# NVlabs/ODISE

Hardware: AMD Instinct MI355X
Metric: panoptic-inference images/sec @1024x1024 (higher is better)
Workload: dtype f16

## Files before the change

odise_amd/csrc/gemm.hip:

```cpp
#include "common.h"
#include <stdlib.h>
#include <type_traits>

#ifdef ODISE_TOOLS
#define ODISE_ABLATE(g, bit) ((g).dbg & (bit))
#else
#define ODISE_ABLATE(g, bit) false
#endif

namespace odise {

struct GemmEpi {
    void* C;
    int64_t ldc;
    int c_dtype;
    const float* bias_n;
    const float* bias_m;
    const float* scale_m;
    const f16* residual;
    int64_t ldr;
    const float* rowgroup_add;
    int rows_per_group;
    int64_t ldg;
    int act;
// ... 1949 lines not shown
    };
    auto finish = [&](TileK& t) { t.kw = (t.ky * 3 + t.kx) * g.cg.Cin + t.chunk * BK; };
    auto advance = [&](TileK& t) {
        if (++t.kx == 3) {
            t.kx = 0;
            if (++t.ky == 3) { t.ky = 0; ++t.chunk; }
        }
        finish(t);
    };

    AccBlock acc[TM][TN];
#pragma unroll
    for (int i = 0; i < TM; ++i)
#pragma unroll
        for (int j = 0; j < TN; ++j) acc_zero(acc[i][j]);

    const int lrow = Frag::lrow(lane), lkq = Frag::lk(lane);
    int koff[Frag::NSTEP];
#pragma unroll
    for (int s = 0; s < Frag::NSTEP; ++s) koff[s] = (Frag::kslot(s, lkq) ^ ((lrow >> 1) & 7)) << 4;
    const int b_lane_off = (wn * WTN + lrow) * 128;
    const int a_pix0 = (wm * 4 + (lrow >> 4)) * HW_ + (lrow & 15);

    auto read_a = [&](const TileK& t, int s, f16x8 (&dst)[TM][Frag::NSTEP][Frag::PER]) {
        const char* ha = smem + HALO0 + (t.chunk & 1) * HALO_BYTES;
        const int pix = a_pix0 + t.ky * HW_ + t.kx;
        const int key = (((lrow & 15) + t.kx) >> 1) & 7;
#pragma unroll
        for (int i = 0; i < TM; ++i)
#pragma unroll
            for (int u = 0; u < Frag::PER; ++u)
                dst[i][s][u] = *reinterpret_cast<const f16x8*>(ha + (pix + (i * 2 + u) * HW_) * 128 + ((Frag::kslot(s, lkq) ^ key) << 4));
    };
    TileK t0;
    t0.ky = t0.kx = 0;
    t0.chunk = kt_begin / 9;
    finish(t0);
    TileK t1 = t0, t2;
    if (kt_begin < kt_end) {
        advance(t1);
        issue_halo(t0.chunk);
#pragma unroll
        for (int j = 0; j < JB; ++j) issue_B(j, 0, t0.kw);
        if (kt_begin + 1 < kt_end) {
#pragma unroll
            for (int j = 0; j < LB; ++j) issue_B(j, 1, t1.kw);
            wait_vmcnt<LB>();
        } else {
            wait_vmcnt<0>();
        }
    }
    t2 = t1;
    advance(t2);
    __builtin_amdgcn_s_barrier();
    TileK tc = t0;
    f16x8 af[TM][Frag::NSTEP][Frag::PER], bf[PT][Frag::NSTEP][Frag::PER];
    {
        const char* fb = smem + b_lane_off;
#pragma unroll
        for (int s = 0; s < Frag::NSTEP; ++s) {
            read_a(tc, s, af);
#pragma unroll
            for (int jj = 0; jj < PT; ++jj)
#pragma unroll
                for (int u = 0; u < Frag::PER; ++u) bf[jj][s][u] = *reinterpret_cast<const f16x8*>(fb + koff[s] + jj * 4096 + u * 2048);
        }
    }
    if (grp == 1) __builtin_amdgcn_s_barrier();

    for (int kt = kt_begin; kt < kt_end; ++kt) {
        const int cur = (kt - kt_begin) & 1;
        const bool has1 = (kt + 1) < kt_end, has2 = (kt + 2) < kt_end;
        const bool opens = tc.ky == 0 && tc.kx == 0;
        const bool halo_next = opens && (kt + 9) < kt_end;
#pragma unroll
        for (int p = 0; p < NP; ++p) {
            const int j0 = PT * p;
            if (p == 0) {
                if (has1) {
#pragma unroll
                    for (int j = LB; j < JB; ++j) issue_B(j, cur ^ 1, t1.kw);
                }
                if (halo_next) issue_halo(tc.chunk + 1);
                if (halo_next) { if (has1) wait_vmcnt<LB + H>(); else wait_vmcnt<H>(); }
                else { if (has1) wait_vmcnt<LB>(); else wait_vmcnt<0>(); }
            } else {
                if (has2) {
#pragma unroll
                    for (int j = 0; j < LB; ++j) issue_B(j, cur, t2.kw);
                }
                if (halo_next) { if (has2) wait_vmcnt<LB + H>(); else wait_vmcnt<H>(); }
                else { if (has2) wait_vmcnt<LB>(); else wait_vmcnt<0>(); }
            }
            asm volatile("s_waitcnt lgkmcnt(0)" ::: "memory");
            __builtin_amdgcn_sched_barrier(0);
            __builtin_amdgcn_s_barrier();
            __builtin_amdgcn_sched_barrier(0);
            const bool next_in_tile = (p + 1 < NP);
            const bool have_next = next_in_tile || has1;
            const char* nfb = smem + (next_in_tile ? cur : (cur ^ 1)) * B_BYTES + b_lane_off + (next_in_tile ? (j0 + PT) * 4096 : 0);
            __builtin_amdgcn_s_setprio(1);
#pragma unroll
            for (int s = 0; s < Frag::NSTEP; ++s) {
#pragma unroll
                for (int jj = 0; jj < PT; ++jj)
#pragma unroll
                    for (int i = 0; i < TM; ++i) mma_step(acc[i][j0 + jj], bf[jj][s], af[i][s]);
                if (have_next) {
                    if (!next_in_tile) read_a(t1, s, af);
#pragma unroll
                    for (int jj = 0; jj < PT; ++jj)
#pragma unroll
                        for (int u = 0; u < Frag::PER; ++u) bf[jj][s][u] = *reinterpret_cast<const f16x8*>(nfb + koff[s] + jj * 4096 + u * 2048);
                }
            }
            __builtin_amdgcn_s_setprio(0);
            __builtin_amdgcn_sched_barrier(0);
            __builtin_amdgcn_s_barrier();
            __builtin_amdgcn_sched_barrier(0);
        }
        tc = t1;
        t1 = t2;
        advance(t2);
    }
    if (grp == 0) __builtin_amdgcn_s_barrier();
    asm volatile("s_waitcnt vmcnt(0) lgkmcnt(0)" ::: "memory");
    __syncthreads();
    gemm_epilogue<BM, BN, WAVES_M, WAVES_N, epi_wave_rows(BM, BN, WAVES_M, halo_lds_bytes(BN)), true, true, true,
                  epi16_rows_if_enabled(BM, BN, WAVES_M, halo_lds_bytes(BN)), false, halo_lds_bytes(BN)>(g, acc, smem, m0, n0, z, zb, split);
}

template <int BN>
__global__ void __launch_bounds__(256, 2) conv3_halo4_kernel(GemmArgs g) {
    constexpr int BM = 256, BK = 64, WAVES_M = 4, WAVES_N = 1;
    constexpr int TM = 2, TN = BN / 32;
    constexpr int JB = BN / 32;
    constexpr int HW_ = 18, HPIX = HW_ * HW_;
    constexpr int HGROUPS = (HPIX + 7) / 8;
    constexpr int H = 11;
    constexpr int B_BYTES = BN * BK * 2;
    constexpr int HALO0 = 2 * B_BYTES;
    extern __shared__ __attribute__((aligned(16))) char smem[];

    const int tid = threadIdx.x;
    const int lane = tid & 63;
    const int wave = __builtin_amdgcn_readfirstlane(tid >> 6);
    const int wm = wave;
    const int hi = lane >> 5, l31 = lane & 31;
    int bx, by;
    {
        const int nbx = gridDim.x, nb = gridDim.x * gridDim.y;
        const int bid = blockIdx.y * nbx + blockIdx.x;
        const int q = nb >> 3, r = nb & 7;
        const int xcd = bid & 7, idx = bid >> 3;
        const int logical = (xcd < r ? xcd * (q + 1) : r * (q + 1) + (xcd - r) * q) + idx;
        by = logical / nbx;
        bx = logical - by * nbx;
    }
    const int m0 = by * BM;
    const int n0 = bx * BN;
    const int z = blockIdx.z;
    const bool split = g.splitk > 1;
    const int zb = 0;
    const int nk_total = g.K / BK;
    int kt_begin = 0, kt_end = nk_total;
    if (split) {
        kt_begin = z * g.ktiles_per_split;
        kt_end = kt_begin + g.ktiles_per_split;
        if (kt_end > nk_total) kt_end = nk_total;
    }
    const f16* Wb = g.W;
    const int per_img = g.cg.halo_tx * g.cg.halo_ty;
    const int img = by / per_img, pr = by - img * per_img;
    const int py0 = (pr / g.cg.halo_tx) * 16 - 1, px0 = (pr % g.cg.halo_tx) * 16 - 1;
    const f16* Ab = g.A + (int64_t)img * g.cg.H * g.cg.W * g.cg.Cin;

    int h_off[H];
#pragma unroll
    for (int h = 0; h < H; ++h) {
        const int group = h * 4 + wave;
        const int hp = group * 8 + (lane >> 3);
        h_off[h] = -1;
        if (group < HGROUPS && hp < HPIX) {
            const int hy = hp / HW_, hx = hp - hy * HW_;
            const int iy = py0 + hy, ix = px0 + hx;
            const int up = g.cg.ups ? 1 : 0;
            if ((unsigned)iy < (unsigned)(g.cg.H << up) && (unsigned)ix < (unsigned)(g.cg.W << up))
                h_off[h] = ((iy >> up) * g.cg.W + (ix >> up)) * g.cg.Cin + (((lane & 7) ^ ((hx >> 1) & 7)) << 3);
        }
    }
    auto issue_halo = [&](int chunk) {
#pragma unroll
        for (int h = 0; h < H; ++h) {
            const int group = h * 4 + wave;
            const f16* src = h_off[h] >= 0 ? Ab + h_off[h] + chunk * BK : g.zeros;
            glds16(src, smem + HALO0 + (group < HGROUPS ? group : HGROUPS) * 1024);
        }
    };
    const int rb = wave * 8 + (lane >> 3);
    const int ls = (lane & 7) ^ ((rb >> 1) & 7);
    const int64_t b_off0 = (int64_t)(n0 + rb) * g.ldw + ls * 8;
    auto issue_B = [&](int stage, int kw) {
#pragma unroll
        for (int j = 0; j < JB; ++j) {
            const bool ok = (n0 + rb + 32 * j) < g.N;
            const f16* src = ok ? Wb + b_off0 + (int64_t)(32 * j) * g.ldw + kw : g.zeros;
            glds16(src, smem + stage * B_BYTES + (32 * j + wave * 8) * 128);
        }
    };

    AccBlock acc[TM][TN];
#pragma unroll
    for (int i = 0; i < TM; ++i)
#pragma unroll
        for (int j = 0; j < TN; ++j) acc_zero(acc[i][j]);

    const int lrow = Frag::lrow(lane), lkq = Frag::lk(lane);
    int koff[Frag::NSTEP];
#pragma unroll
    for (int s = 0; s < Frag::NSTEP; ++s) koff[s] = (Frag::kslot(s, lkq) ^ ((lrow >> 1) & 7)) << 4;
    const int b_lane_off = lrow * 128;
    const int a_pix0 = (wm * 4 + (lrow >> 4)) * HW_ + (lrow & 15);

    int ky = 0, kx = 0, chunk = kt_begin / 9;
    if (kt_begin < kt_end) {
        issue_halo(chunk);
        issue_B(0, chunk * BK);
    }
    for (int kt = kt_begin; kt < kt_end; ++kt) {
        const int cur = (kt - kt_begin) & 1;
        asm volatile("s_waitcnt vmcnt(0)" ::: "memory");
        __builtin_amdgcn_s_barrier();
        int nky = ky, nkx = kx + 1, nchunk = chunk;
        if (nkx == 3) { nkx = 0; if (++nky == 3) { nky = 0; ++nchunk; } }
        const bool more = kt + 1 < kt_end;
        if (more) issue_B(cur ^ 1, (nky * 3 + nkx) * g.cg.Cin + nchunk * BK);
        const char* ha = smem + HALO0;
        const char* fb = smem + cur * B_BYTES + b_lane_off;
        const int pix = a_pix0 + ky * HW_ + kx;
        const int key = (((lrow & 15) + kx) >> 1) & 7;
        f16x8 af[2][TM][Frag::PER], bf[2][TN][Frag::PER];
        auto read_frags = [&](int s, int b) {
#pragma unroll
            for (int u = 0; u < Frag::PER; ++u) {
#pragma unroll
                for (int i = 0; i < TM; ++i) af[b][i][u] = *reinterpret_cast<const f16x8*>(ha + (pix + (i * 2 + u) * HW_) * 128 + ((Frag::kslot(s, lkq) ^ key) << 4));
#pragma unroll
                for (int j = 0; j < TN; ++j) bf[b][j][u] = *reinterpret_cast<const f16x8*>(fb + koff[s] + j * 4096 + u * 2048);
            }
        };
        read_frags(0, 0);
#pragma unroll
        for (int s = 0; s < Frag::NSTEP; ++s) {
            if (s + 1 < Frag::NSTEP) read_frags(s + 1, (s + 1) & 1);
            __builtin_amdgcn_sched_barrier(0);
#pragma unroll
            for (int j = 0; j < TN; ++j)
#pragma unroll
                for (int i = 0; i < TM; ++i) mma_step(acc[i][j], bf[s & 1][j], af[s & 1][i]);
            __builtin_amdgcn_sched_barrier(0);
        }
        if (more && nchunk != chunk) {
            asm volatile("s_waitcnt lgkmcnt(0)" ::: "memory");
            __builtin_amdgcn_s_barrier();
            issue_halo(nchunk);
        }
        ky = nky; kx = nkx; chunk = nchunk;
    }
    asm volatile("s_waitcnt vmcnt(0) lgkmcnt(0)" ::: "memory");
    __syncthreads();
    gemm_epilogue<BM, BN, WAVES_M, WAVES_N, epi_wave_rows(BM, BN, WAVES_M, halo4_lds_bytes(BN)), true, true, true,
                  epi16_rows_if_enabled(BM, BN, WAVES_M, halo4_lds_bytes(BN)), false, halo4_lds_bytes(BN)>(g, acc, smem, m0, n0, z, zb, split);
}

__global__ void __launch_bounds__(256) splitk_reduce_kernel(const float* __restrict__ ws, int splitk, int M, int N, GemmEpi e) {
    const int CH = (N + 7) / 8;
    const int64_t total = (int64_t)M * CH;
    const bool vec = (N & 3) == 0;
    for (int64_t idx = (int64_t)blockIdx.x * blockDim.x + threadIdx.x; idx < total; idx += (int64_t)gridDim.x * blockDim.x) {
        const int m = (int)(idx / CH);
        const int n = (int)(idx - (int64_t)m * CH) * 8;
        const int nv = (N - n) < 8 ? (N - n) : 8;
        float v[8];
#pragma unroll
        for (int i = 0; i < 8; ++i) v[i] = 0.f;
        if (vec && nv == 8) {
            for (int s = 0; s < splitk; ++s) {
                const float4* w = reinterpret_cast<const float4*>(ws + ((int64_t)s * M + m) * N + n);
                const float4 a = w[0], b = w[1];
                v[0] += a.x; v[1] += a.y; v[2] += a.z; v[3] += a.w;
                v[4] += b.x; v[5] += b.y; v[6] += b.z; v[7] += b.w;
            }
        } else {
            for (int s = 0; s < splitk; ++s) {
                const float* w = ws + ((int64_t)s * M + m) * N + n;
                for (int i = 0; i < nv; ++i) v[i] += w[i];
            }
        }
        if (e.fast && n + 8 <= N) epi_fast8(e, v, m, n, 0);
        else epi_store8(e, v, m, n, N, 0);
    }
}

static int launch_tile_kernel(odise_hip_ctx* ctx, void (*kern)(GemmArgs), LdsAttrOnce& once, dim3 grid, int threads, int lds, const GemmArgs& g) {
    if (lds > 65536) ODISE_TRY(ensure_dyn_lds(ctx, once, (const void*)kern, lds));
    hipLaunchKernelGGL(kern, grid, dim3(threads), lds, ctx->stream, g);
    ODISE_CHECK_HIP(hipGetLastError());
    if (g.splitk > 1) {
        const int64_t total = (int64_t)g.M * ceil_div(g.N, 8);
        const int blocks = (int)std::min<int64_t>(ceil_div(total, 256), 2048);
        hipLaunchKernelGGL(splitk_reduce_kernel, dim3(blocks), dim3(256), 0, ctx->stream, g.ws, g.splitk, g.M, g.N, g.epi);
        ODISE_CHECK_HIP(hipGetLastError());
    }
    return ODISE_OK;
}
static dim3 gemm_grid(const GemmArgs& g, int BM, int BN, int batch) {
    return dim3((unsigned)ceil_div(g.N, BN), (unsigned)ceil_div(g.M, BM), (unsigned)(g.splitk > 1 ? g.splitk : batch));
}
static dim3 halo_grid(const GemmArgs& g, int BN) {
    const int n_img = g.M / (g.cg.OH * g.cg.OW);
    return dim3((unsigned)ceil_div(g.N, BN), (unsigned)(n_img * g.cg.halo_tx * g.cg.halo_ty), (unsigned)(g.splitk > 1 ? g.splitk : 1));
}

template <int BM, int BN, int WAVES_M, int WAVES_N, bool CONV>
static int launch_gemm_t(odise_hip_ctx* ctx, GemmArgs& g, int batch) {
    constexpr int lds = plain_lds_bytes(BM, BN, WAVES_M);
    static_assert(epi_lds_bytes(BM, BN, WAVES_M, epi_wave_rows(BM, BN, WAVES_M, lds)) <= lds, "epilogue staging exceeds the LDS request");
    static LdsAttrOnce once;
    return launch_tile_kernel(ctx, gemm_kernel<BM, BN, WAVES_M, WAVES_N, CONV>, once, gemm_grid(g, BM, BN, batch), 64 * WAVES_M * WAVES_N, lds, g);
}

template <int BM, int BN, int WAVES_N, int PT, bool CONV>
static int launch_gemm_pp(odise_hip_ctx* ctx, GemmArgs& g, int batch) {
    constexpr int lds = pp_lds_bytes(BM, BN, 8 / WAVES_N);
    static_assert(epi_lds_bytes(BM, BN, 8 / WAVES_N, epi_wave_rows(BM, BN, 8 / WAVES_N, lds)) <= lds, "epilogue staging exceeds the LDS request");
    static_assert(lds > 65536, "the ping-pong tiles always opt in to dynamic LDS");
    static LdsAttrOnce once;
    return launch_tile_kernel(ctx, gemm_pp_kernel<BM, BN, WAVES_N, PT, CONV>, once, gemm_grid(g, BM, BN, batch), 512, lds, g);
}

template <int BM, int BN, int WAVES_N, int PT, bool CONV>
static int launch_gemm_pp2(odise_hip_ctx* ctx, GemmArgs& g, int batch) {
    static_assert((BN / WAVES_N / 32) % PT == 0, "whole phases");
    constexpr int lds = pp_lds_bytes(BM, BN, 8 / WAVES_N);
    static_assert(lds > 65536, "the ping-pong tiles always opt in to dynamic LDS");
    static LdsAttrOnce once;
    return launch_tile_kernel(ctx, gemm_pp2_kernel<BM, BN, WAVES_N, PT, CONV>, once, gemm_grid(g, BM, BN, batch), 512, lds, g);
}

template <int BN, int PT>
static int launch_conv3_halo(odise_hip_ctx* ctx, GemmArgs& g) {
    constexpr int lds = halo_lds_bytes(BN);
    static_assert(epi_lds_bytes(256, BN, 4, epi_wave_rows(256, BN, 4, lds)) <= lds, "epilogue staging exceeds the LDS request");
    static_assert(lds > 65536, "the halo tiles always opt in to dynamic LDS");
    static LdsAttrOnce once;
    return launch_tile_kernel(ctx, conv3_halo_kernel<BN, PT>, once, halo_grid(g, BN), 512, lds, g);
}

template <int BN>
static int launch_conv3_halo4(odise_hip_ctx* ctx, GemmArgs& g) {
    constexpr int lds = halo4_lds_bytes(BN);
    static_assert(2 * lds <= 160 * 1024, "two blocks must fit a CU's LDS");
    static_assert(epi_lds_bytes(256, BN, 4, epi_wave_rows(256, BN, 4, lds)) <= lds, "epilogue staging exceeds the LDS request");
    static_assert(lds > 65536, "the halo tiles always opt in to dynamic LDS");
    static LdsAttrOnce once;
    return launch_tile_kernel(ctx, conv3_halo4_kernel<BN>, once, halo_grid(g, BN), 256, lds, g);
}

static int g_gemm_debug = 0;
enum SelectFlag : int {
    kFlagNoPingPong = 2,
    kFlagNo512x128 = 16,
    kFlagLaunchLog = 32,
    kFlagNoHalo = 64,
    kFlagForcePP2 = 512,
    kFlagNoPP2 = 1024,
    kFlagNoHalo4 = 2048,
    kFlagBlockEpilogue = 32768,
    kFlagNoHaloUpsample = 131072,
};
static int g_conv_flags = 0;

enum Tile : int {
    kTile128x128 = 0, kTile64x128 = 1, kTile64x64 = 2, kTile256x320 = 3, kTile256x256 = 4, kTile256x128 = 5, kTile512x128 = 6,
    kTileHalo256 = 7, kTileHalo128 = 8, kTileHalo128x4 = 9, kNumTiles = 10
};
static bool is_halo_tile(int t) { return t >= kTileHalo256 && t <= kTileHalo128x4; }
static bool has_pingpong_form(int t) { return t == kTile256x320 || t == kTile256x256 || t == kTile512x128; }
static const int kTileBM[kNumTiles] = {128, 64, 64, 256, 256, 256, 512, 256, 256, 256};
static const int kTileBN[kNumTiles] = {128, 128, 64, 320, 256, 128, 128, 256, 128, 128};

struct TileCost {
    double t_ktile, t_fixed;
    int slots_per_cu;
};
static const TileCost kTileCost[kNumTiles] = {
    {1.45, 6.0, 2},
    {1.25, 3.5, 3},
    {1.06, 2.6, 4},
    {2.65, 15.0, 1},
    {2.10, 15.0, 1},
    {1.42, 6.0, 1},
    {2.25, 12.0, 1},
    {1.47, 22.5, 1},
    {1.12, 9.0, 1},
    {1.70, 12.0, 2},
};
static const TileCost kTileCostPP[2] = {
    {2.00, 16.0, 1},
    {1.56, 10.0, 1},
};
static const TileCost kTileCostConv512 = {2.5, 16.0, 1};
static const TileCost kTileCostPPConv256 = {1.49, 25.5, 1};
static thread_local int g_last_tile = -1;
static int env_gemm_flags() {
#ifdef ODISE_TOOLS
    static int v = -1;
    if (v < 0) {
        const char* e = getenv("ODISE_GEMM_FLAGS");
        v = e ? atoi(e) : 0;
    }
    return v;
#else
    return 0;
#endif
}

template <bool CONV>
static int launch_gemm_select(odise_hip_ctx* ctx, GemmArgs& g, int batch, int force_tile, int force_split, unsigned tile_mask);

template <bool CONV>
static int launch_gemm(odise_hip_ctx* ctx, GemmArgs& g, int batch, int force_tile, int force_split, unsigned tile_mask = ~0u) {
    LaunchProbe* pr = probe_match(ctx, CONV, g.M, g.N, g.K);
    if (pr && CONV && g.cg.ups) pr = nullptr;
    if (pr) {
        hipStreamCaptureStatus st = hipStreamCaptureStatusNone;
        if (hipStreamIsCapturing(ctx->stream, &st) != hipSuccess || st != hipStreamCaptureStatusNone) pr = nullptr;
    }
    if (!pr) return launch_gemm_select<CONV>(ctx, g, batch, force_tile, force_split, tile_mask);
    const int i = pr->n;
    const bool started = hipEventRecord(pr->ev[2 * i], ctx->stream) == hipSuccess;
    const int rc = launch_gemm_select<CONV>(ctx, g, batch, force_tile, force_split, tile_mask);
    if (started && hipEventRecord(pr->ev[2 * i + 1], ctx->stream) == hipSuccess) pr->n = i + 1;
    else { (void)hipGetLastError(); pr->armed = false; }
    return rc;
}

static int select_flags() { return g_conv_flags | env_gemm_flags(); }
template <bool CONV>
static int launch_gemm_select(odise_hip_ctx* ctx, GemmArgs& g, int batch, int force_tile, int force_split, unsigned tile_mask) {
    const int64_t cus = ctx->cu_count;
    const int nk = (int)ceil_div(g.K, 64);
    bool halo_ok = false;
    int64_t halo_patches = 0;
    if (CONV) {
        const int up = g.cg.ups ? 1 : 0;
        halo_ok = g.cg.KH == 3 && g.cg.KW == 3 && g.cg.stride == 1 && g.cg.pad_t == 1 && g.cg.pad_l == 1 && g.cg.Cin % 64 == 0 &&
                  g.cg.OH == (g.cg.H << up) && g.cg.OW == (g.cg.W << up) && batch == 1 && !(up && (select_flags() & kFlagNoHaloUpsample));
        g.cg.halo_tx = (int)ceil_div(g.cg.OW, 16);
        g.cg.halo_ty = (int)ceil_div(g.cg.OH, 16);
        halo_patches = (int64_t)(g.M / (g.cg.OH * g.cg.OW)) * g.cg.halo_tx * g.cg.halo_ty;
    }
    auto blocks = [&](int t) {
        return (is_halo_tile(t) ? halo_patches : ceil_div(g.M, kTileBM[t])) * ceil_div(g.N, kTileBN[t]) * (int64_t)batch;
    };
    int tile = kTile64x64, best_split = 1;
    double best = 1e30;
    const int flags = select_flags();
    const bool pp_base = !(flags & kFlagNoPingPong) && g.K % 64 == 0 && (!CONV || g.cg.Cin % 64 == 0);
    const bool pp_ok = pp_base && !(CONV && g.cg.ups);
    for (int t = 0; t < kNumTiles; ++t) {
        if (force_tile >= 0 && force_tile < kNumTiles && t != force_tile) continue;
        if (!((tile_mask >> t) & 1)) continue;
        if (t == kTile512x128 && (!pp_ok || (flags & kFlagNo512x128))) continue;
        if (is_halo_tile(t) && (!halo_ok || !pp_base || (flags & kFlagNoHalo))) continue;
        if (t == kTileHalo128x4 && (flags & kFlagNoHalo4)) continue;
        if (t == kTileHalo128x4 && force_tile < 0 && g.N > 128) continue;
        const TileCost& tc = (CONV && pp_ok && t == kTile256x256) ? kTileCostPPConv256 :
                             (pp_ok && (t == kTile256x320 || t == kTile256x256)) ? kTileCostPP[t - kTile256x320] :
                             (CONV && t == kTile512x128) ? kTileCostConv512 : kTileCost[t];
        if (force_tile < 0) {
            if (kTileBM[t] > 64 && g.M <= kTileBM[t] / 2) continue;
            if (kTileBN[t] > 64 && g.N <= kTileBN[t] / 2 && t != kTile64x64) continue;
        }
        const int64_t nb = blocks(t);
        const int64_t slots = cus * tc.slots_per_cu;
        const int max_split = (batch == 1) ? std::max(1, std::min(nk / 2, 32)) : 1;
        for (int sp = 1; sp <= max_split; ++sp) {
            if (force_split > 0 && sp != std::min(force_split, std::max(1, nk))) continue;
            if (sp > 1 && (size_t)sp * g.M * g.N * sizeof(float) > ctx->ws_bytes) break;
            const int per = is_halo_tile(t) ? (int)ceil_div(nk / 9, sp) * 9 : (int)ceil_div(nk, sp);
            const int eff_sp = (int)ceil_div(nk, per);
            const int64_t nblk = nb * eff_sp;
            const int64_t rounds = ceil_div(nblk, slots);
            const double fill_last = (double)(nblk - (rounds - 1) * slots) / (double)slots;
            double t_us = per * tc.t_ktile * ((double)(rounds - 1) + 0.55 + 0.45 * fill_last) + (double)rounds * tc.t_fixed;
            if (eff_sp > 1) t_us += 4.0 + ((2.0 * eff_sp * 4.0 + 2.0) * (double)g.M * g.N) / 6.0e6;
            if (t_us < best) { best = t_us; tile = t; best_split = eff_sp; }
        }
    }
    if (force_tile >= 0 && force_tile < kNumTiles && !(force_tile == kTile512x128 && !pp_ok) && !(is_halo_tile(force_tile) && !(halo_ok && pp_base)))
        tile = force_tile;
    g.splitk = 1;
    g.ktiles_per_split = nk;
    if (force_split > 0 && batch == 1) best_split = std::min(force_split, nk);
    if (best_split > 1 && batch == 1) {
        g.ktiles_per_split = is_halo_tile(tile) ? (int)ceil_div(nk / 9, best_split) * 9 : (int)ceil_div(nk, best_split);
        g.splitk = (int)ceil_div(nk, g.ktiles_per_split);
        ODISE_REQUIRE((size_t)g.splitk * g.M * g.N * sizeof(float) <= ctx->ws_bytes, "gemm: split-K workspace too small");
    }
    g_last_tile = tile | (best_split << 8);
    if (ctx->launch_log) launch_log_push(ctx, LaunchRec{(int)CONV, g.M, g.N, g.K, tile, g.splitk});
    if (flags & kFlagLaunchLog) {
        fprintf(stderr, "GEMMLOG conv=%d M=%d N=%d K=%d batch=%d cin=%d kh=%d h=%d w=%d stride=%d ups=%d tile=%d split=%d pp=%d\n", (int)CONV, g.M, g.N,
                g.K, batch, g.cg.Cin, g.cg.KH, g.cg.H, g.cg.W, g.cg.stride, g.cg.ups, tile, best_split, (int)pp_ok);
    }
    g.ws = (float*)ctx->ws;
    {
        const GemmEpi& e = g.epi;
        const int esz = e.c_dtype == ODISE_F16 ? 2 : 4;
        const int out_vec = (e.geglu ? 4 : 8) * esz;
        auto aligned = [](const void* p, int64_t ld_elems, int64_t stride_elems, int elem, int bytes) {
            return ((uintptr_t)p % bytes) == 0 && (ld_elems * elem) % bytes == 0 && (stride_elems * elem) % bytes == 0;
        };
        bool ok = aligned(e.C, e.ldc, e.strideC, esz, out_vec);
        ok = ok && (!e.residual || (!e.geglu && aligned(e.residual, e.ldr, e.strideR, 2, 16)));
        ok = ok && (!e.bias_n || ((uintptr_t)e.bias_n & 15) == 0);
        ok = ok && (!e.rowgroup_add || (((uintptr_t)e.rowgroup_add & 15) == 0 && e.ldg % 4 == 0));
        ok = ok && (!e.geglu || e.act == ODISE_ACT_NONE);
        g.epi.fast = ok ? 1 : 0;
        const int n_out = e.geglu ? g.N / 2 : g.N;
        g.epi.f16path = (ok && e.c_dtype == ODISE_F16 && g.N % 8 == 0 && n_out % 8 == 0 && aligned(e.C, e.ldc, e.strideC, 2, 16) &&
                         (!e.residual || aligned(e.residual, e.ldr, e.strideR, 2, 8))) ? 1 : 0;
    }
    if (g.epi.ln_part || g.epi.ln_final || g.epi.ln_stats_out) {
        ODISE_REQUIRE(!CONV && (tile == kTile256x256 || tile == kTile256x128) && g.splitk == 1 && g.epi.f16path && !g.epi.geglu && batch == 1 &&
                          (!g.epi.ln_stats_out || (tile == kTile256x256 && g.N % kLnPartCols == 0)),
                      "gemm_ln: M=%d N=%d K=%d cannot take the folded-LayerNorm path", g.M, g.N, g.K);
    }
    g.stats_blocks = 0;
    if (g.epi.gn_stats) {
        const int ohw = CONV ? g.cg.OH * g.cg.OW : 0;
        const bool pp2_used = (tile == kTile256x256) && pp_ok && ((flags & kFlagForcePP2) || (!(flags & kFlagNoPP2) && CONV));
        bool ok = CONV && g.splitk == 1 && g.epi.fast && g.N % 8 == 0 &&
                  (is_halo_tile(tile) || (tile == kTile512x128 && pp_ok && !(flags & kFlagForcePP2)) || pp2_used);
        if (ok && is_halo_tile(tile)) g.stats_blocks = g.cg.halo_tx * g.cg.halo_ty;
        else if (ok && ohw % kTileBM[tile] == 0) g.stats_blocks = ohw / kTileBM[tile];
        else ok = false;
        if (!ok) { g.epi.gn_stats = nullptr; g.stats_blocks = 0; }
    }
    g.zeros = (const f16*)ctx->zeros;
    g.epi_block = (flags & kFlagBlockEpilogue) ? 1 : 0;
#ifdef ODISE_TOOLS
    static const int freeze_k = (getenv("ODISE_GEMM_FREEZE_K") ? 16 : 0) | (getenv("ODISE_NO_RES_PREFETCH") ? 64 : 0);
    g.dbg = g_gemm_debug | freeze_k;
#else
    g.dbg = 0;
#endif
    if (is_halo_tile(tile)) {
        g.cg.chunk_major = 1;
        if (tile == kTileHalo128x4) return launch_conv3_halo4<128>(ctx, g);
        return tile == kTileHalo256 ? launch_conv3_halo<256, 2>(ctx, g) : launch_conv3_halo<128, 1>(ctx, g);
    }
    g.cg.halo_tx = g.cg.halo_ty = 0;
    const bool pp2_auto = !(flags & kFlagNoPP2) && ((CONV && tile != kTile512x128) || (!CONV && blocks(tile) * (g.splitk > 1 ? g.splitk : 1) <= 2 * cus));
    if (has_pingpong_form(tile) && pp_ok && ((flags & kFlagForcePP2) || pp2_auto)) {
        if (tile == kTile512x128) return launch_gemm_pp2<512, 128, 1, 2, CONV>(ctx, g, batch);
        if (tile == kTile256x320) return launch_gemm_pp2<256, 320, 2, 1, CONV>(ctx, g, batch);
        return launch_gemm_pp2<256, 256, 2, 2, CONV>(ctx, g, batch);
    }
    if (has_pingpong_form(tile) && pp_ok) {
        if (tile == kTile512x128) return launch_gemm_pp<512, 128, 1, 2, CONV>(ctx, g, batch);
        if (tile == kTile256x320) return launch_gemm_pp<256, 320, 2, 1, CONV>(ctx, g, batch);
        return launch_gemm_pp<256, 256, 2, 2, CONV>(ctx, g, batch);
    }
    switch (tile) {
        case kTile128x128: return launch_gemm_t<128, 128, 2, 2, CONV>(ctx, g, batch);
        case kTile64x128: return launch_gemm_t<64, 128, 2, 2, CONV>(ctx, g, batch);
        case kTile256x320: return launch_gemm_t<256, 320, 4, 2, CONV>(ctx, g, batch);
        case kTile256x256: return launch_gemm_t<256, 256, 4, 2, CONV>(ctx, g, batch);
        case kTile256x128: return launch_gemm_t<256, 128, 4, 2, CONV>(ctx, g, batch);
        default: return launch_gemm_t<64, 64, 2, 2, CONV>(ctx, g, batch);
    }
}

int conv_forced(odise_hip_ctx* ctx, const odise_conv_desc* d, int force_tile, int force_split, float* gn_stats = nullptr, int* stats_blocks = nullptr);

int gemm_forced(odise_hip_ctx* ctx, const odise_gemm_desc* d, int force_tile, int force_split, const LnEpi* ln) {
    ODISE_REQUIRE(ctx && d, "gemm: null argument");
    ODISE_REQUIRE(d->M >= 0 && d->N >= 0 && d->K > 0, "gemm: bad dims M=%d N=%d K=%d", d->M, d->N, d->K);
    if (d->M == 0 || d->N == 0) return ODISE_OK;
    ODISE_REQUIRE(d->K % 8 == 0, "gemm: K=%d must be a multiple of 8", d->K);
    ODISE_REQUIRE(d->lda % 8 == 0 && d->ldw % 8 == 0, "gemm: lda/ldw must be multiples of 8 (16-byte rows)");
    ODISE_REQUIRE(((uintptr_t)d->A & 15) == 0 && ((uintptr_t)d->W & 15) == 0, "gemm: A/W must be 16-byte aligned");
    ODISE_REQUIRE(d->A && d->W && d->C, "gemm: null device pointer");
    ODISE_REQUIRE(d->c_dtype == ODISE_F16 || d->c_dtype == ODISE_F32, "gemm: bad c_dtype");
    ODISE_REQUIRE(!d->geglu || (d->N % 2 == 0), "gemm: geglu needs even N");
    ODISE_REQUIRE(!d->rowgroup_add || d->rows_per_group > 0, "gemm: rows_per_group must be > 0");
    const int batch = d->batch < 1 ? 1 : d->batch;
    ODISE_REQUIRE(batch == 1 || ((d->strideA % 8 == 0) && (d->strideW % 8 == 0)), "gemm: batch strides must keep 16-byte alignment");
    GemmArgs g;
    g.M = d->M; g.N = d->N; g.K = d->K;
    g.A = (const f16*)d->A; g.lda = d->lda; g.strideA = d->strideA;
    g.W = (const f16*)d->W; g.ldw = d->ldw; g.strideW = d->strideW;
    g.epi.C = d->C; g.epi.ldc = d->ldc; g.epi.c_dtype = d->c_dtype;
    g.epi.bias_n = d->bias_n; g.epi.bias_m = d->bias_m; g.epi.scale_m = d->scale_m;
    g.epi.residual = (const f16*)d->residual; g.epi.ldr = d->ldr;
    g.epi.rowgroup_add = d->rowgroup_add; g.epi.rows_per_group = d->rows_per_group > 0 ? d->rows_per_group : 1;
    g.epi.ldg = d->ldg > 0 ? d->ldg : d->N;
    g.epi.act = d->act; g.epi.geglu = d->geglu; g.epi.alpha = d->alpha;
    g.epi.strideC = d->strideC; g.epi.strideR = d->strideR;
    if (ln) {
        g.epi.ln_part = ln->part; g.epi.ln_P = ln->P; g.epi.ln_inv_c = ln->inv_c; g.epi.ln_eps = ln->eps; g.epi.ln_colsum = ln->colsum;
        g.epi.ln_final_out = ln->final_out; g.epi.ln_final = ln->fin; g.epi.ln_rowsum = ln->rowsum; g.epi.ln_stats_out = ln->stats_out;
        ODISE_REQUIRE((!ln->part || (ln->P > 0 && ln->colsum)) && (!ln->fin || ln->rowsum), "gemm_ln: incomplete LayerNorm terms");
    }
    g.cg = ConvGeom{};
    if (ln) return launch_gemm<false>(ctx, g, batch, force_tile, 1, ln->stats_out ? (1u << kTile256x256) : (1u << kTile256x256) | (1u << kTile256x128));
    return launch_gemm<false>(ctx, g, batch, force_tile, force_split);
}

int gemm_ln(odise_hip_ctx* ctx, const odise_gemm_desc* d, const LnEpi& ln) { return gemm_forced(ctx, d, -1, 1, &ln); }

int conv_forced(odise_hip_ctx* ctx, const odise_conv_desc* d, int force_tile, int force_split, float* gn_stats, int* stats_blocks) {
    ODISE_REQUIRE(ctx && d, "conv2d: null argument");
    ODISE_REQUIRE(d->N >= 0 && d->H > 0 && d->W > 0 && d->Cin > 0 && d->Cout > 0, "conv2d: bad dims");
    ODISE_REQUIRE(d->Cin % 8 == 0, "conv2d: Cin=%d must be a multiple of 8 (pad the input channels)", d->Cin);
    ODISE_REQUIRE(d->KH >= 1 && d->KW >= 1 && d->stride >= 1 && d->OH > 0 && d->OW > 0, "conv2d: bad kernel geometry");
    ODISE_REQUIRE(d->X && d->Wt && d->Y, "conv2d: null device pointer");
    ODISE_REQUIRE(((uintptr_t)d->X & 15) == 0 && ((uintptr_t)d->Wt & 15) == 0, "conv2d: X/Wt must be 16-byte aligned");
    if (d->N == 0) return ODISE_OK;
    if (force_tile < 0 && force_split <= 0 && conv3_c8_ok(d)) return launch_conv3_c8(ctx, d, gn_stats, stats_blocks);
    GemmArgs g;
    g.M = d->N * d->OH * d->OW;
    g.N = d->Cout;
    g.K = d->KH * d->KW * d->Cin;
    g.A = (const f16*)d->X; g.lda = 0; g.strideA = 0;
    g.W = (const f16*)d->Wt; g.ldw = g.K; g.strideW = 0;
    g.epi.C = d->Y; g.epi.ldc = d->Cout; g.epi.c_dtype = d->y_dtype;
    g.epi.bias_n = d->bias; g.epi.bias_m = nullptr; g.epi.scale_m = nullptr;
    g.epi.residual = (const f16*)d->residual; g.epi.ldr = d->Cout;
    g.epi.rowgroup_add = d->per_image_add; g.epi.rows_per_group = d->OH * d->OW;
    g.epi.ldg = d->per_image_add_ld > 0 ? d->per_image_add_ld : d->Cout;
    g.epi.act = d->act; g.epi.geglu = 0; g.epi.alpha = 1.0f;
    g.epi.strideC = 0; g.epi.strideR = 0;
    g.epi.gn_stats = gn_stats;
    if (stats_blocks) *stats_blocks = 0;
    g.cg.H = d->H; g.cg.W = d->W; g.cg.Cin = d->Cin; g.cg.KH = d->KH; g.cg.KW = d->KW;
    g.cg.stride = d->stride; g.cg.pad_t = d->pad_t; g.cg.pad_l = d->pad_l; g.cg.OH = d->OH; g.cg.OW = d->OW;
    g.cg.ups = d->upsample2x;
    const int64_t in_bytes = (int64_t)d->N * d->H * d->W * d->Cin * 2;
    g.cg.chunk_major = (d->Cin % 64 == 0 && d->KH * d->KW > 1 && in_bytes <= (128ll << 20)) ? 1 : 0;
    if (d->KH == 1 && d->KW == 1 && d->stride == 1 && d->pad_t == 0 && d->pad_l == 0 && !d->upsample2x && d->OH == d->H &&
        d->OW == d->W) {
        g.lda = d->Cin;
        return launch_gemm<false>(ctx, g, 1, force_tile, force_split);
    }
    const int rc = launch_gemm<true>(ctx, g, 1, force_tile, force_split);
    if (stats_blocks) *stats_blocks = (rc == ODISE_OK) ? g.stats_blocks : 0;
    return rc;
}

int group_norm_from_colpart(odise_hip_ctx* ctx, const void* x, void* y, const float* gamma, const float* beta, int N, int HW, int C, int groups,
                            float eps, int act, const float* colpart, int nblk);

}

extern "C" int odise_hip_gemm_debug(int flags) {
    odise::g_gemm_debug = flags & 15;
    odise::g_conv_flags = (flags >> 4) & 0xfffff;
    return 0;
}
extern "C" int odise_hip_gemm(odise_hip_ctx* ctx, const odise_gemm_desc* d) { return odise::gemm_forced(ctx, d, -1, 0); }
extern "C" int odise_hip_conv2d(odise_hip_ctx* ctx, const odise_conv_desc* d) { return odise::conv_forced(ctx, d, -1, 0); }
extern "C" int odise_hip_gemm_forced(odise_hip_ctx* ctx, const odise_gemm_desc* d, int tile, int splitk) {
    return odise::gemm_forced(ctx, d, tile, splitk);
}
extern "C" int odise_hip_last_tile(void) { return odise::g_last_tile; }
extern "C" int odise_hip_gemm_ln(odise_hip_ctx* ctx, const odise_gemm_desc* d, const float* part, int parts, float inv_c, float eps,
                                 const float* colsum, float* final_out, const float* fin, const float* rowsum, float* stats_out) {
    odise::LnEpi ln;
    ln.part = part; ln.P = parts; ln.inv_c = inv_c; ln.eps = eps; ln.colsum = colsum; ln.final_out = final_out;
    ln.fin = fin; ln.rowsum = rowsum; ln.stats_out = stats_out;
    return odise::gemm_ln(ctx, d, ln);
}
extern "C" int odise_hip_conv2d_forced(odise_hip_ctx* ctx, const odise_conv_desc* d, int tile, int splitk) {
    return odise::conv_forced(ctx, d, tile, splitk);
}
extern "C" int odise_hip_conv2d_gn_forced(odise_hip_ctx* ctx, const odise_conv_desc* d, int tile, int splitk, const float* gamma, const float* beta,
                                          int groups, float eps, int act, void* y_norm, float* stats_scratch, int* stats_blocks) {
    ODISE_REQUIRE(ctx && d && gamma && beta && y_norm && stats_scratch && stats_blocks, "conv2d_gn_forced: null argument");
    ODISE_REQUIRE(d->y_dtype == ODISE_F16, "conv2d_gn_forced: f16 output only");
    if (int rc = odise::conv_forced(ctx, d, tile, splitk, stats_scratch, stats_blocks)) return rc;
    if (*stats_blocks > 0)
        return odise::group_norm_from_colpart(ctx, d->Y, y_norm, gamma, beta, d->N, d->OH * d->OW, d->Cout, groups, eps, act, stats_scratch, *stats_blocks);
    return odise_hip_group_norm(ctx, d->Y, y_norm, gamma, beta, d->N, d->OH * d->OW, d->Cout, groups, eps, act);
}
```

Baseline: 53.43.

## Add in-block split-K skinny GEMM kernel that folds partials through LDS

```diff
diff --git a/odise_amd/csrc/gemm.hip b/odise_amd/csrc/gemm.hip
--- a/odise_amd/csrc/gemm.hip
+++ b/odise_amd/csrc/gemm.hip
@@ -2275,6 +2275,151 @@
     }
 }
 
+template <int BM, int BN, int NW, int STAGES>
+__global__ void __launch_bounds__(64 * NW) gemm_skinny_kernel(GemmArgs g) {
+    using FL = FragLayout;
+    constexpr int BK = 64;
+    constexpr int NT = 64 * NW;
+    constexpr int TM = BM / 32, TN = BN / 32;
+    constexpr int JA = BM / 8, JB = BN / 8, NL = JA + JB;
+    constexpr int STAGE_BYTES = (BM + BN) * BK * 2;
+    constexpr int LDS_LD = BN + 4, CH = BN / 8;
+    constexpr int FOLD_FLOATS = BM * LDS_LD;
+    constexpr int IT = (BM * CH + NT - 1) / NT;
+    static_assert(BM % 32 == 0 && BN % 32 == 0 && STAGES >= 1 && STAGES <= 3 && (STAGES - 1) * NL < 64, "bad skinny tile");
+    extern __shared__ __attribute__((aligned(16))) char smem[];
+
+    const int tid = threadIdx.x;
+    const int lane = tid & 63;
+    const int wave = __builtin_amdgcn_readfirstlane(tid >> 6);
+    const int m0 = blockIdx.y * BM, n0 = blockIdx.x * BN;
+    const int nk_total = (g.K + BK - 1) / BK;
+    char* wbase = smem + wave * (STAGES * STAGE_BYTES);
+
+    const int slot = lane & 7, r8 = lane >> 3;
+    const f16* a_row = g.A + (int64_t)(m0 + r8) * g.lda;
+    const f16* w_row = g.W + (int64_t)(n0 + r8) * g.ldw;
+    auto issue_tile = [&](int kt, int stage) {
+        char* sa = wbase + stage * STAGE_BYTES;
+        char* sb = sa + BM * BK * 2;
+        const int k_even = kt * BK + ((slot ^ (lane >> 4)) << 3), k_odd = kt * BK + ((slot ^ ((lane >> 4) + 4)) << 3);
+#pragma unroll
+        for (int j = 0; j < JA; ++j) {
+            const int k = (j & 1) ? k_odd : k_even;
+            const f16* src = (m0 + r8 + 8 * j < g.M && k < g.K) ? a_row + (int64_t)(8 * j) * g.lda + k : g.zeros;
+            glds16(src, sa + j * 1024);
+        }
+#pragma unroll
+        for (int j = 0; j < JB; ++j) {
+            const int k = (j & 1) ? k_odd : k_even;
+            const f16* src = (n0 + r8 + 8 * j < g.N && k < g.K) ? w_row + (int64_t)(8 * j) * g.ldw + k : g.zeros;
+            glds16(src, sb + j * 1024);
+        }
+    };
+    const int lrow = Frag::lrow(lane), lkq = Frag::lk(lane);
+    int koff[Frag::NSTEP];
+#pragma unroll
+    for (int s = 0; s < Frag::NSTEP; ++s) koff[s] = (Frag::kslot(s, lkq) ^ ((lrow >> 1) & 7)) << 4;
+
+    float v[IT][8];
+#pragma unroll
+    for (int it = 0; it < IT; ++it)
+#pragma unroll
+        for (int i = 0; i < 8; ++i) v[it][i] = 0.f;
+
+    const int rounds = (g.splitk + NW - 1) / NW;
+    for (int r = 0; r < rounds; ++r) {
+        const int s = r * NW + wave;
+        AccBlock acc[TM][TN];
+#pragma unroll
+        for (int i = 0; i < TM; ++i)
+#pragma unroll
+            for (int j = 0; j < TN; ++j) acc_zero(acc[i][j]);
+        if (s < g.splitk) {
+            const int kt_begin = s * g.ktiles_per_split;
+            const int n = (kt_begin + g.ktiles_per_split < nk_total ? kt_begin + g.ktiles_per_split : nk_total) - kt_begin;
+#pragma unroll
+            for (int i = 0; i < STAGES - 1; ++i)
+                if (i < n) issue_tile(kt_begin + i, i);
+            int cur = 0, nxt = STAGES - 1;
+            for (int i = 0; i < n; ++i) {
+                asm volatile("s_waitcnt lgkmcnt(0)" ::: "memory");
+                if (i + STAGES - 1 < n) issue_tile(kt_begin + i + STAGES - 1, nxt);
+                const int after = (n - 1 - i) < (STAGES - 1) ? (n - 1 - i) : (STAGES - 1);
+                if (STAGES == 3 && after == 2) wait_vmcnt<2 * NL>();
+                else if (STAGES >= 2 && after == 1) wait_vmcnt<NL>();
+                else wait_vmcnt<0>();
+                const char* fa = wbase + cur * STAGE_BYTES + lrow * 128;
+                const char* fb = fa + BM * BK * 2;
+                f16x8 af[TM][Frag::PER], bf[TN][Frag::PER];
+#pragma unroll
+                for (int st = 0; st < Frag::NSTEP; ++st) {
+#pragma unroll
+                    for (int i2 = 0; i2 < TM; ++i2)
+#pragma unroll
+                        for (int u = 0; u < Frag::PER; ++u) af[i2][u] = *reinterpret_cast<const f16x8*>(fa + koff[st] + i2 * 4096 + u * 2048);
+#pragma unroll
+                    for (int j = 0; j < TN; ++j)
+#pragma unroll
+                        for (int u = 0; u < Frag::PER; ++u) bf[j][u] = *reinterpret_cast<const f16x8*>(fb + koff[st] + j * 4096 + u * 2048);
+#pragma unroll
+                    for (int i2 = 0; i2 < TM; ++i2)
+#pragma unroll
+                        for (int j = 0; j < TN; ++j) mma_step(acc[i2][j], bf[j], af[i2]);
+                }
+                cur = (cur + 1 == STAGES) ? 0 : cur + 1;
+                nxt = (nxt + 1 == STAGES) ? 0 : nxt + 1;
+            }
+        }
+        __syncthreads();
+        float* stg = reinterpret_cast<float*>(smem);
+        if (s < g.splitk) {
+            float* mine = stg + wave * FOLD_FLOATS;
+#pragma unroll
+            for (int p = 0; p < TM; ++p)
+#pragma unroll
+                for (int j = 0; j < TN; ++j)
+#pragma unroll
+                    for (int rr = 0; rr < FL::NR; ++rr)
+#pragma unroll
+                        for (int q = 0; q < FL::NC; ++q) {
+                            const int r0 = 4 * (rr * FL::NC + q);
+                            *reinterpret_cast<float4*>(&mine[(p * 32 + FL::row(lane, rr)) * LDS_LD + j * 32 + FL::col(lane, q)]) =
+                                make_float4(acc_get(acc, p, j, r0), acc_get(acc, p, j, r0 + 1), acc_get(acc, p, j, r0 + 2), acc_get(acc, p, j, r0 + 3));
+                        }
+        }
+        __syncthreads();
+        const int ns = (g.splitk - r * NW) < NW ? (g.splitk - r * NW) : NW;
+#pragma unroll
+        for (int it = 0; it < IT; ++it) {
+            const int c = tid + it * NT;
+            if ((BM * CH) % NT != 0 && c >= BM * CH) continue;
+            const int row = c / CH, c8 = c - row * CH;
+            for (int q = 0; q < ns; ++q) {
+                const float4 t0 = *reinterpret_cast<const float4*>(&stg[q * FOLD_FLOATS + row * LDS_LD + c8 * 8]);
+                const float4 t1 = *reinterpret_cast<const float4*>(&stg[q * FOLD_FLOATS + row * LDS_LD + c8 * 8 + 4]);
+                v[it][0] += t0.x; v[it][1] += t0.y; v[it][2] += t0.z; v[it][3] += t0.w;
+                v[it][4] += t1.x; v[it][5] += t1.y; v[it][6] += t1.z; v[it][7] += t1.w;
+            }
+        }
+        if (r + 1 < rounds) __syncthreads();
+    }
+#pragma unroll
+    for (int it = 0; it < IT; ++it) {
+        const int c = tid + it * NT;
+        if ((BM * CH) % NT != 0 && c >= BM * CH) continue;
+        const int row = c / CH, c8 = c - row * CH;
+        const int m = m0 + row, n = n0 + c8 * 8;
+        if (m < g.M && n < g.N) {
+            if (g.epi.fast && n + 8 <= g.N) epi_fast8(g.epi, v[it], m, n, 0);
+            else epi_store8(g.epi, v[it], m, n, g.N, 0);
+        }
+    }
+}
+constexpr int skinny_lds_bytes(int BM, int BN, int NW, int STAGES) {
+    return max_int(NW * STAGES * (BM + BN) * 64 * 2, NW * BM * (BN + 4) * 4);
+}
+
 static int launch_tile_kernel(odise_hip_ctx* ctx, void (*kern)(GemmArgs), LdsAttrOnce& once, dim3 grid, int threads, int lds, const GemmArgs& g) {
     if (lds > 65536) ODISE_TRY(ensure_dyn_lds(ctx, once, (const void*)kern, lds));
     hipLaunchKernelGGL(kern, grid, dim3(threads), lds, ctx->stream, g);
@@ -2338,6 +2483,18 @@
     static_assert(lds > 65536, "the halo tiles always opt in to dynamic LDS");
     static LdsAttrOnce once;
     return launch_tile_kernel(ctx, conv3_halo4_kernel<BN>, once, halo_grid(g, BN), 256, lds, g);
+}
+
+template <int BM, int BN, int NW, int STAGES>
+static int launch_gemm_skinny(odise_hip_ctx* ctx, GemmArgs& g) {
+    constexpr int lds = skinny_lds_bytes(BM, BN, NW, STAGES);
+    static_assert(lds <= 160 * 1024, "the skinny tile's stages exceed a CU's LDS");
+    static LdsAttrOnce once;
+    void (*kern)(GemmArgs) = gemm_skinny_kernel<BM, BN, NW, STAGES>;
+    if (lds > 65536) ODISE_TRY(ensure_dyn_lds(ctx, once, (const void*)kern, lds));
+    hipLaunchKernelGGL(kern, dim3((unsigned)ceil_div(g.N, BN), (unsigned)ceil_div(g.M, BM), 1), dim3(64 * NW), lds, ctx->stream, g);
+    ODISE_CHECK_HIP(hipGetLastError());
+    return ODISE_OK;
 }
 
 static int g_gemm_debug = 0;
@@ -2351,6 +2508,7 @@
     kFlagNoHalo4 = 2048,
     kFlagBlockEpilogue = 32768,
     kFlagNoHaloUpsample = 131072,
+    kFlagNoSkinny = 262144,
 };
 static int g_conv_flags = 0;
 
@@ -2358,6 +2516,8 @@
     kTile128x128 = 0, kTile64x128 = 1, kTile64x64 = 2, kTile256x320 = 3, kTile256x256 = 4, kTile256x128 = 5, kTile512x128 = 6,
     kTileHalo256 = 7, kTileHalo128 = 8, kTileHalo128x4 = 9, kNumTiles = 10
 };
+enum : int { kTileSkinny = 10, kNumSkinnyForms = 2 };
+static const int kSkinnyMaxM = 512;
 static bool is_halo_tile(int t) { return t >= kTileHalo256 && t <= kTileHalo128x4; }
 static bool has_pingpong_form(int t) { return t == kTile256x320 || t == kTile256x256 || t == kTile512x128; }
 static const int kTileBM[kNumTiles] = {128, 64, 64, 256, 256, 256, 512, 256, 256, 256};
@@ -2482,11 +2642,18 @@
         g.splitk = (int)ceil_div(nk, g.ktiles_per_split);
         ODISE_REQUIRE((size_t)g.splitk * g.M * g.N * sizeof(float) <= ctx->ws_bytes, "gemm: split-K workspace too small");
     }
-    g_last_tile = tile | (best_split << 8);
-    if (ctx->launch_log) launch_log_push(ctx, LaunchRec{(int)CONV, g.M, g.N, g.K, tile, g.splitk});
+    int skinny = 0;
+    if (!CONV && batch == 1 && g.M <= kSkinnyMaxM && !(g.epi.ln_part || g.epi.ln_final || g.epi.ln_stats_out)) {
+        if (force_tile > kTileSkinny && force_tile <= kTileSkinny + kNumSkinnyForms) skinny = force_tile - kTileSkinny + 1;
+        else if (force_tile == kTileSkinny || (force_tile < 0 && force_split <= 0 && g.splitk > 1 && tile <= kTile64x64 && !(flags & kFlagNoSkinny)))
+            skinny = 1;
+    }
+    const int tile_id = skinny ? (int)kTileSkinny : tile;
+    g_last_tile = tile_id | (best_split << 8);
+    if (ctx->launch_log) launch_log_push(ctx, LaunchRec{(int)CONV, g.M, g.N, g.K, tile_id, g.splitk});
     if (flags & kFlagLaunchLog) {
         fprintf(stderr, "GEMMLOG conv=%d M=%d N=%d K=%d batch=%d cin=%d kh=%d h=%d w=%d stride=%d ups=%d tile=%d split=%d pp=%d\n", (int)CONV, g.M, g.N,
-                g.K, batch, g.cg.Cin, g.cg.KH, g.cg.H, g.cg.W, g.cg.stride, g.cg.ups, tile, best_split, (int)pp_ok);
+                g.K, batch, g.cg.Cin, g.cg.KH, g.cg.H, g.cg.W, g.cg.stride, g.cg.ups, tile_id, best_split, (int)pp_ok);
     }
     g.ws = (float*)ctx->ws;
     {
@@ -2530,6 +2697,10 @@
 #else
     g.dbg = 0;
 #endif
+    if (skinny) {
+        const bool eight = skinny == 1 ? g.splitk > 4 : skinny == 3;
+        return eight ? launch_gemm_skinny<32, 64, 8, 1>(ctx, g) : launch_gemm_skinny<32, 64, 4, 3>(ctx, g);
+    }
     if (is_halo_tile(tile)) {
         g.cg.chunk_major = 1;
         if (tile == kTileHalo128x4) return launch_conv3_halo4<128>(ctx, g);
```

Result: no change. 53.40, median of 2 (-0.0%).
